# tsunrise/r1cs-spartan

Measured on AMD Instinct MI355X. Metric: R1CS constraints proved/sec at 2^20, higher is better.
Workload: dtype bls12-381 Fr/Fq Montgomery (u32 limbs)

## Files before the change

### include/spartan_hip.h

```cpp
#ifndef SPARTAN_HIP_H
#define SPARTAN_HIP_H
#include <stddef.h>
#include <stdint.h>

#ifdef __cplusplus
extern "C" {
#endif

typedef enum {
    SPX_OK = 0,
    SPX_INVALID_ARGUMENT = 1,
    SPX_SUMCHECK = 2,
    SPX_WRONG_WITNESS = 3,
    SPX_SERIALIZATION = 4,
    SPX_DEVICE = 5
} spx_status;

typedef struct spx_ctx spx_ctx;
typedef struct spx_pp spx_pp;
typedef struct spx_pk spx_pk;
typedef struct spx_witness spx_witness;

typedef struct {
    uint64_t n;
// ... 129 lines not shown
    SPX_K_RED_G1 = 11,
    SPX_K_RED_G2 = 12,
    SPX_K_COUNT = 13
};
int spx_kernel_stats_enable(spx_ctx *ctx, int on);
int spx_kernel_stats(spx_ctx *ctx, int id, uint64_t *launches, double *ms, double *bytes);
int spx_kernel_stats_largest(spx_ctx *ctx, int id, uint64_t *launches, double *ms, double *bytes);
int spx_kernel_ops(spx_ctx *ctx, int id, double *ops);
int spx_msm_reruns(spx_ctx *ctx, uint64_t *reruns);

int spx_msm_skew_stats(spx_ctx *ctx, uint64_t out[4]);

int spx_msm_window_plan(uint64_t size, int *c, int *windows);
int spx_msm_level_plan(int nv, int *c);
int spx_pp_window_plan(spx_pp *pp, int level, int *c, int *windows);

int spx_sum_over_y(spx_ctx *ctx, const spx_csr *m, const uint8_t *z, uint8_t *out);
int spx_eval_on_x(spx_ctx *ctx, const spx_csr *m, const uint8_t *r_x, uint8_t *out);
int spx_sumcheck_round(spx_ctx *ctx, const uint8_t *f, const uint8_t *g, size_t n, const uint8_t *r_prev,
                       uint8_t *evals_out, uint8_t *f_out, uint8_t *g_out);
int spx_msm_g1(spx_ctx *ctx, const uint8_t *bases, const uint8_t *scalars, size_t n, uint8_t *out96);
int spx_msm_g2(spx_ctx *ctx, const uint8_t *bases, const uint8_t *scalars, size_t n, uint8_t *out192);
int spx_g1_decompress(spx_ctx *ctx, const uint8_t *in, size_t n, uint8_t *out_uncompressed, uint8_t *ok);
int spx_g2_decompress(spx_ctx *ctx, const uint8_t *in, size_t n, uint8_t *out_uncompressed, uint8_t *ok);
int spx_lincomb_g1(spx_ctx *ctx, const uint8_t *bases_uncompressed, const uint8_t *scalars, size_t n,
                   const uint64_t *seg_off, size_t nseg, uint8_t *out_uncompressed);
int spx_lincomb_g2(spx_ctx *ctx, const uint8_t *bases_uncompressed, const uint8_t *scalars, size_t n,
                   const uint64_t *seg_off, size_t nseg, uint8_t *out_uncompressed);
int spx_g1_in_subgroup(spx_ctx *ctx, const uint8_t *pts_uncompressed, size_t n, uint8_t *ok);
int spx_g2_in_subgroup(spx_ctx *ctx, const uint8_t *pts_uncompressed, size_t n, uint8_t *ok);
// ... 16 lines not shown
```

### r1cs-spartan_amd/__init__.py

```python
import ctypes
import os

_HERE = os.path.dirname(os.path.abspath(__file__))
LIB_PATH = os.environ.get("SPX_LIB_PATH") or os.path.join(_HERE, "libspartan_hip.so")

R = 0x73EDA753299D7D483339D80809A1D80553BDA402FFFE5BFEFFFFFFFF00000001


class SpartanError(Exception):
    code = -1


class InvalidArgument(SpartanError):
    code = 1


class SumCheckError(SpartanError):
    code = 2


class WrongWitness(SpartanError):
    code = 3


# ... 41 lines not shown
    "spx_ctx_set_msm_hot",
    "spx_comm_hub_create_rccl",
    "spx_comm_hub_create_shm",
    "spx_comm_hub_create_group",
    "spx_comm_hub_create_callback",
    "spx_ctx_set_comm_hub",
    "spx_comm_hub_allgather",
    "spx_comm_hub_stats",
    "spx_comm_hub_destroy",
    "spx_ctx_comm_allgather",
    "spx_msm_reruns",
    "spx_msm_skew_stats",
    "spx_msm_window_plan",
    "spx_msm_level_plan",
    "spx_pp_window_plan",
    "spx_ctx_mem_info",
    "spx_ctx_set_sync_poll",
    "spx_ctx_set_group",
    "spx_host_phase_stats",
    "spx_pp_load",
    "spx_pp_generate",
    "spx_pp_serialize",
    "spx_pp_free",
    "spx_index",
    "spx_index_free",
    "spx_witness_upload",
    "spx_witness_free",
    "spx_proof_size",
    "spx_prove",
    "spx_prove_witness",
# ... 81 lines not shown
        L.spx_ctx_set_sync_poll.argtypes = [vp, ctypes.c_int]
    if hasattr(L, "spx_ctx_set_group") or not os.environ.get("SPX_LIB_PATH"):
        L.spx_ctx_set_group.argtypes = [vp, ctypes.c_int]
    if hasattr(L, "spx_ctx_mem_info") or not os.environ.get("SPX_LIB_PATH"):
        L.spx_ctx_mem_info.argtypes = [vp, ctypes.POINTER(ctypes.c_uint64), ctypes.POINTER(ctypes.c_uint64)]
    if hasattr(L, "spx_ctx_set_lvl0_batch"):
        L.spx_ctx_set_lvl0_batch.argtypes = [vp, ctypes.c_int]
    if hasattr(L, "spx_ctx_set_msm_hot") or not os.environ.get("SPX_LIB_PATH"):
        L.spx_ctx_set_msm_hot.argtypes = [vp, ctypes.c_int]
        L.spx_msm_skew_stats.argtypes = [vp, ctypes.POINTER(ctypes.c_uint64)]
    if hasattr(L, "spx_msm_window_plan") or not os.environ.get("SPX_LIB_PATH"):
        pint = ctypes.POINTER(ctypes.c_int)
        L.spx_msm_window_plan.argtypes = [ctypes.c_uint64, pint, pint]
        L.spx_msm_level_plan.argtypes = [ctypes.c_int, pint]
        L.spx_pp_window_plan.argtypes = [vp, ctypes.c_int, pint, pint]
    if hasattr(L, "spx_comm_hub_create_rccl") or not os.environ.get("SPX_LIB_PATH"):
        L.spx_comm_hub_create_rccl.argtypes = [u8p, ctypes.c_int, ctypes.c_int, ctypes.c_int, ctypes.POINTER(vp)]
        L.spx_comm_hub_create_shm.argtypes = [ctypes.c_char_p, ctypes.c_int, ctypes.c_int, ctypes.POINTER(vp)]
        L.spx_comm_hub_create_group.argtypes = [vp, ctypes.c_int, ctypes.POINTER(vp)]
        if hasattr(L, "spx_comm_hub_create_callback") or not os.environ.get("SPX_LIB_PATH"):
            L.spx_comm_hub_create_callback.argtypes = [ALLGATHER_FN, vp, ctypes.c_int, ctypes.c_int, ctypes.POINTER(vp)]
        L.spx_ctx_set_comm_hub.argtypes = [vp, vp, ctypes.c_int]
        L.spx_comm_hub_allgather.argtypes = [vp, ctypes.c_int, ctypes.c_char_p, ctypes.c_void_p, sz]
        L.spx_comm_hub_stats.argtypes = [vp, ctypes.c_void_p]
        L.spx_comm_hub_destroy.argtypes = [vp]
    L.spx_ctx_comm_allgather.argtypes = [vp, ctypes.c_char_p, ctypes.c_void_p, sz]
    L.spx_pp_load.argtypes = [vp, u8p, sz, ctypes.POINTER(vp)]
    L.spx_pp_generate.argtypes = [vp, ctypes.c_int, ctypes.c_uint64, ctypes.POINTER(vp)]
    L.spx_pp_serialize.argtypes = [vp, ctypes.c_void_p, sz, ctypes.POINTER(sz)]
    L.spx_pp_free.argtypes = [vp]
# ... 370 lines not shown
    def check_subgroup(self, strict=True):
        bad = ctypes.c_uint64(0)
        first = (ctypes.c_uint64 * 3)()
        rc = lib().spx_pp_check_subgroup(self.ctx.h, self.h, ctypes.byref(bad), first)
        if rc != 0 and (strict or rc != 4):
            _check(rc)
        if bad.value == 0:
            return 0, None
        return bad.value, (int(first[0]), None if first[1] == 2**64 - 1 else int(first[1]), int(first[2]))

    def window_plan(self, level):
        c, w = ctypes.c_int(0), ctypes.c_int(0)
        _check(lib().spx_pp_window_plan(self.h, int(level), ctypes.byref(c), ctypes.byref(w)))
        return c.value, w.value

    def serialize_uncompressed(self):
        n = ctypes.c_size_t(0)
        _check(lib().spx_pp_serialize(self.h, None, 0, ctypes.byref(n)))
        buf = ctypes.create_string_buffer(n.value)
        _check(lib().spx_pp_serialize(self.h, buf, n.value, ctypes.byref(n)))
        return buf.raw

    def __del__(self):
        try:
            if self.h and self.ctx.h:
                lib().spx_pp_free(self.h)
        except Exception:
            pass


# ... 479 lines not shown
```

### r1cs-spartan_amd/csrc/capi.cpp

```cpp
#include "../../include/spartan_hip.h"

#include <atomic>
#include <chrono>
#include <algorithm>
#include <cstdlib>
#include <mutex>
#include <condition_variable>
#include <memory>
#include <string>
#include <thread>
#include <vector>

#include "hash_sched.hpp"
#include "interactive.hpp"
#include "pairing.hpp"
#include "prover.hpp"

extern "C" int spx_comm_unique_id_impl(uint8_t out[128]);

struct spx_ctx {
    std::unique_ptr<spx::Ctx> c;
};
struct spx_pp {
    spx_ctx* ctx;
// ... 269 lines not shown
    });
}
int spx_pp_serialize(spx_pp* pp, uint8_t* out, size_t cap, size_t* len) {
    return guard([&] {
        set_dev(pp->ctx);
        copy_out(spx::pp_serialize(*pp->ctx->c, *pp->p), out, cap, len);
    });
}
int spx_pp_window_plan(spx_pp* pp, int level, int* c, int* windows) {
    return guard([&] {
        if (!pp || !c || !windows) spx::invalid("null argument");
        const spx::PP& P = *pp->p;
        if (level < -1 || level >= P.nv) spx::invalid("level out of range");
        *c = level < 0 ? P.g1_c : P.g2_c[level];
        *windows = level < 0 ? P.g1_W : P.g2_W[level];
    });
}
int spx_msm_window_plan(uint64_t size, int* c, int* windows) {
    return guard([&] {
        if (!c || !windows) spx::invalid("null argument");
        *c = spx::window_bits_for(size, spx::msm_wide_min_log());
        *windows = spx::windows_for(*c);
    });
}
int spx_msm_level_plan(int nv, int* c) {
    return guard([&] {
        if (!c) spx::invalid("null argument");
        if (nv < 1 || nv > spx::kMaxLogN) spx::invalid("nv out of range");
        const std::vector<int> plan = spx::g2_window_plan(nv, spx::msm_wide_min_log());
        std::copy(plan.begin(), plan.end(), c);
// ... 619 lines not shown
```

### r1cs-spartan_amd/csrc/curve_dev.hpp

```cpp
#pragma once
#include "ff_dev.hpp"

namespace spx {

template <class F>
struct Aff {
    F x, y;
};
template <class F>
struct Xyzz {
    F x, y, zz, zzz;
};
using G1Aff = Aff<Fq>;
struct G1Slot {
    G1Aff p;
    uint32_t pad[8];
};
static_assert(sizeof(G1Slot) == 128, "G1 table slot");
using G2Aff = Aff<Fq2>;
using G1Xyzz = Xyzz<Fq>;
using G2Xyzz = Xyzz<Fq2>;

template <class F>
DEV void xyzz_set_inf(Xyzz<F>& p) {
    FieldOps<F>::one(p.x);
    FieldOps<F>::one(p.y);
    FieldOps<F>::zero(p.zz);
    FieldOps<F>::zero(p.zzz);
}
template <class F>
DEV bool xyzz_is_inf(const Xyzz<F>& p) {
    return FieldOps<F>::is_zero(p.zz);
}

// ... 159 lines not shown
```

### r1cs-spartan_amd/csrc/kernels.hpp

```cpp
#pragma once
#include <hip/hip_runtime.h>
#include <stdint.h>

#include <vector>

#include "curve_dev.hpp"

namespace spx {

static constexpr uint64_t kLongRow = 64;
static constexpr uint64_t kChunk = 4096;

struct SparseView3 {
    const uint64_t* ptr[3];
    const uint32_t* idx[3];
    const Fr* val[3];
};
struct LongChunk {
    uint32_t m;
    uint32_t pad;
    uint64_t begin, end;
};
struct LongRow {
    uint32_t m;
// ... 202 lines not shown
static constexpr uint32_t kMsmOverflow = 1;
enum { kMsmStHot = 1, kMsmStReduced = 2, kMsmStLeafMax = 3 };

static constexpr uint64_t kMsmMaxBuckets = 2048ull << 8;
static constexpr uint32_t kMsmWideBits = 17, kMsmWideWindows = 15;
static constexpr uint32_t msm_windows(uint32_t c) { return c == kMsmWideBits ? kMsmWideWindows : (256 + c - 1) / c; }
struct MsmWorkspace;
MsmWorkspace* msm_ws_create();
void msm_ws_destroy(MsmWorkspace* ws);
void msm_ws_staging_reset(MsmWorkspace* ws);
void msm_ws_note_overflow(MsmWorkspace* ws);
void msm_ws_set_hot(MsmWorkspace* ws, bool on);
bool msm_hot_default();

inline size_t msm_out_bytes(bool g2, int ninst) { return (size_t)ninst * (g2 ? 4 * 96 : 4 * 48) + 16; }
void msm_run_g1(MsmWorkspace* ws, const MsmInst* insts_host, int ninst, const G1Slot* pts, const Fr* scalars,
                void* out_dev, hipStream_t s, const MsmShard& sh = MsmShard());
void msm_run_g2(MsmWorkspace* ws, const MsmInst* insts_host, int ninst, const G2Aff* pts, const Fr* scalars,
                void* out_dev, hipStream_t s, const MsmShard& sh = MsmShard());

void precompute_windows_g1(const G1Aff* raw, uint64_t count, bool pair_sum, int c, int W, G1Aff* dst, void* tmp,
                           hipStream_t s);
void precompute_windows_g2(const G2Aff* raw, uint64_t count, bool pair_sum, int c, int W, G2Aff* dst, void* tmp,
                           hipStream_t s);
void launch_points_from_bytes_g1(G1Aff* pts, uint64_t n, int* err, hipStream_t s);
void launch_points_from_bytes_g2(G2Aff* pts, uint64_t n, int* err, hipStream_t s);
void launch_points_to_canon_g1(G1Aff* pts, uint64_t n, hipStream_t s);
void launch_points_to_canon_g2(G2Aff* pts, uint64_t n, hipStream_t s);
void fixed_base_g1(const G1Aff* table, const Fr* scalars, uint64_t n, G1Aff* out, void* tmp, hipStream_t s);
void fixed_base_g2(const G2Aff* table, const Fr* scalars, uint64_t n, G2Aff* out, void* tmp, hipStream_t s);

void launch_decompress_g1(const uint8_t* in, uint64_t n, G1Aff* out, uint8_t* ok, hipStream_t s);
void launch_decompress_g2(const uint8_t* in, uint64_t n, G2Aff* out, uint8_t* ok, hipStream_t s);
size_t lincomb_tmp_bytes(bool g2, uint64_t n);
void launch_lincomb_g1(const G1Aff* pts, const Fr* scalars, uint64_t n, const uint64_t* seg_off, uint32_t nseg,
                       G1Aff* out, void* tmp, hipStream_t s);
void launch_lincomb_g2(const G2Aff* pts, const Fr* scalars, uint64_t n, const uint64_t* seg_off, uint32_t nseg,
                       G2Aff* out, void* tmp, hipStream_t s);

// ... 7 lines not shown
```

### r1cs-spartan_amd/csrc/msm_g1.hip

```cpp
#include "msm_impl.hpp"

namespace spx {

void msm_run_g1(MsmWorkspace* ws, const MsmInst* insts, int ninst, const G1Slot* pts, const Fr* scalars, void* out,
                hipStream_t s, const MsmShard& sh) {
    msm_run_t<Fq>(ws, insts, ninst, pts, scalars, out, s, sh);
}
void precompute_windows_g1(const G1Aff* raw, uint64_t count, bool pair_sum, int c, int W, G1Aff* dst, void* tmp,
                           hipStream_t s) {
    precompute_windows_t<Fq>(raw, count, pair_sum, c, W, dst, tmp, s);
}
void fixed_base_g1(const G1Aff* table, const Fr* scalars, uint64_t n, G1Aff* out, void* tmp, hipStream_t s) {
    fixed_base_t<Fq>(table, scalars, n, out, tmp, s);
}

}
```

### r1cs-spartan_amd/csrc/msm_g2.hip

```cpp
#include "msm_impl.hpp"

namespace spx {

void msm_run_g2(MsmWorkspace* ws, const MsmInst* insts, int ninst, const G2Aff* pts, const Fr* scalars, void* out,
                hipStream_t s, const MsmShard& sh) {
    msm_run_t<Fq2>(ws, insts, ninst, pts, scalars, out, s, sh);
}
void precompute_windows_g2(const G2Aff* raw, uint64_t count, bool pair_sum, int c, int W, G2Aff* dst, void* tmp,
                           hipStream_t s) {
    precompute_windows_t<Fq2>(raw, count, pair_sum, c, W, dst, tmp, s);
}
void fixed_base_g2(const G2Aff* table, const Fr* scalars, uint64_t n, G2Aff* out, void* tmp, hipStream_t s) {
    fixed_base_t<Fq2>(table, scalars, n, out, tmp, s);
}

}
```

### r1cs-spartan_amd/csrc/msm_impl.hpp

```cpp
#pragma once
#include "curve29.hpp"
#include "fq2pair.hpp"
#include "msm_common.hpp"

namespace spx {

template <class F>
struct Acc;
struct AffRaw {
    Fq x, y;
};
template <>
struct Acc<Fq> {
    using Pt = G1Slot;
    using T = F29;
    using TA = F29;
    static constexpr int kLanes = 1, kWaves = 1;
    static DEV void ld_raw(AffRaw& a, const G1Slot* p) { load_vec(*(Aff<Fq>*)&a, &p->p); }
    static DEV void unpack(T& x, T& y, const AffRaw& a) {
        f29_unpack(x, a.x.v);
        f29_unpack(y, a.y.v);
    }
    static DEV void ld_aff(T& x, T& y, const G1Slot* p) {
        AffRaw a;
        ld_raw(a, p);
        unpack(x, y, a);
    }
    static DEV bool aff_sentinel(const T& x, const T& y) { return f29_is_zero_raw(x) && f29_is_zero_raw(y); }
    static DEV void ld(X29<T>& r, const Xyzz<Fq>* p) { ld29<Fq>(r, p); }
    static DEV void st(Xyzz<Fq>* p, const X29<T>& r) { st29<Fq>(p, r); }
};
template <>
struct Acc<Fq2> {
    using Pt = Aff<Fq2>;
    using T = FP29;
    using TA = FP29A;
    static constexpr int kLanes = 2, kWaves = 2;
    static DEV void ld_raw(AffRaw& a, const Aff<Fq2>* p) {
        const bool odd = pair_odd();
        load_vec(a.x, odd ? &p->x.c1 : &p->x.c0);
        load_vec(a.y, odd ? &p->y.c1 : &p->y.c0);
    }
    template <class P>
    static DEV void unpack(P& x, P& y, const AffRaw& a) {
        f29_unpack(x.v, a.x.v);
        f29_unpack(y.v, a.y.v);
    }
    template <class P>
    static DEV void ld_aff(P& x, P& y, const Aff<Fq2>* p) {
        fp29_ld(x, &p->x);
        fp29_ld(y, &p->y);
    }
    template <class P>
    static DEV bool aff_sentinel(const P& x, const P& y) {
        return pair_all(f29_is_zero_raw(x.v) && f29_is_zero_raw(y.v));
    }
    static DEV void ld(X29<T>& r, const Xyzz<Fq2>* p) {
        fp29_ld(r.x, &p->x);
        fp29_ld(r.y, &p->y);
        fp29_ld(r.zz, &p->zz);
        fp29_ld(r.zzz, &p->zzz);
    }
    template <class P>
    static DEV void st(Xyzz<Fq2>* p, const X29<P>& r) {
        fp29_st(&p->x, r.x);
        fp29_st(&p->y, r.y);
        fp29_st(&p->zz, r.zz);
        fp29_st(&p->zzz, r.zzz);
    }
};
// ... 131 lines not shown
}
template <class F>
static unsigned tree_blocks(uint64_t elems) {
    return (unsigned)((elems * TreeLanes<F>::v + kHeavy - 1) / kHeavy);
}

template <class F>
DEV uint64_t acc_elem() {
    return (blockIdx.x * (uint64_t)blockDim.x + threadIdx.x) / Acc<F>::kLanes;
}
template <class F>
static unsigned acc_blocks(uint64_t elems) {
    return (unsigned)((elems * Acc<F>::kLanes + kHeavy - 1) / kHeavy);
}

template <class F>
__global__ __launch_bounds__(kHeavy, Acc<F>::kWaves) void k_accum_aff(const uint32_t* __restrict__ off, uint32_t nb,
                                                                      const uint32_t* __restrict__ pfx,
                                                                      const uint32_t* __restrict__ refs,
                                                                      const typename Acc<F>::Pt* __restrict__ pts,
                                                                      Xyzz<F>* __restrict__ out, uint32_t seg1) {
    using A = Acc<F>;
    using T = typename A::TA;
    const uint32_t t = (uint32_t)acc_elem<F>();
    const uint32_t total = off[nb];
    uint32_t e = t * seg1;
    if (e >= total) return;
    const uint32_t end = min(e + seg1, total);
    uint32_t b = find_bucket(off, nb, e);
    uint32_t bend = off[b + 1];
    uint32_t slot = pfx[b] + (t - off[b] / seg1);
    X29<T> acc;
    x29_set_inf(acc);
    for (; e < end; ++e) {
        if (e == bend) {
            A::st(out + slot, acc);
            x29_set_inf(acc);
            do {
                ++b;
            } while (off[b + 1] <= e);
            bend = off[b + 1];
            slot = pfx[b];
        }
        const uint32_t r = refs[e];
        T px, py;
        A::ld_aff(px, py, pts + (r & 0x7fffffffu));
        if (A::aff_sentinel(px, py)) continue;
        x29_madd(acc, px, py, (r >> 31) != 0);
    }
    A::st(out + slot, acc);
}

template <class F>
__global__ __launch_bounds__(kHeavy, Acc<F>::kWaves) void k_accum_xyzz(const uint32_t* __restrict__ segoff, uint32_t nb,
                                                                       const uint32_t* __restrict__ off,
                                                                       const Xyzz<F>* __restrict__ in,
                                                                       Xyzz<F>* __restrict__ out) {
    using A = Acc<F>;
    using T = typename A::T;
    const uint32_t s = (uint32_t)tree_elem<F>();
    if (s >= segoff[nb]) return;
    const uint32_t b = find_bucket(segoff, nb, s);
// ... 243 lines not shown
static int msm_levels_env() {
    static const int v = [] {
        const char* e = getenv("SPX_MSM_LEVELS");
        return e ? atoi(e) : -1;
    }();
    return v;
}
static int msm_seg1_env() {
    static const int v = [] {
        const char* e = getenv("SPX_MSM_SEG1");
        return e ? atoi(e) : 0;
    }();
    return v;
}

template <class F>
static void msm_run_t(MsmWorkspace* ws, const MsmInst* ih, int ninst, const typename Acc<F>::Pt* pts, const Fr* scalars,
                      void* out_dev, hipStream_t s, const MsmShard& sh) {
    if (ninst <= 0) return;
    const bool g2 = sizeof(F) == sizeof(Fq2);
    const size_t psz = sizeof(Xyzz<F>);
    const size_t ob = msm_out_bytes(g2, ninst);
    MsmPlan pl = msm_plan(ih, ninst, sh, ws->cap_scale);
    const int nact = (int)pl.insts.size();
    if (!nact) {
        HIPCHK(hipMemsetAsync(out_dev, 0, ob, s));
        return;
    }
    msm_upload_plan(ws, pl, s);
    const uint32_t nb = pl.nb;
    const uint64_t tot_refs = pl.tot_refs;
    uint32_t kSeg1 = seg1_fit(seg1_len(g2), tot_refs, Acc<F>::kWaves, Acc<F>::kLanes);
    if (msm_seg1_env() > 0) kSeg1 = std::min<uint32_t>(kSeg1, (uint32_t)msm_seg1_env());
    const double mu = pl.mu_max;
    int nlev = 0;
    for (uint32_t m = (uint32_t)std::ceil((mu + 6.0 * std::sqrt(mu) + 16.0) / kSeg1) + 1; m > 1; m = (m + kSeg - 1) / kSeg)
        ++nlev;
    if (msm_levels_env() >= 0) nlev = std::min(nlev, msm_levels_env());
    MsmSorted so = msm_sort(ws, pl, scalars, out_dev, ob, s, kSeg1, nlev);
    const uint64_t max_segs = tot_refs / kSeg1 + nb + 1;
    auto* PA = (Xyzz<F>*)ws->pa.ensure(psz * max_segs);
    auto* PB = (Xyzz<F>*)ws->pb.ensure(psz * (max_segs / kSeg + nb + 1));
    uint32_t* cur_off = so.np_off;
    uint32_t* nxt_off = nullptr;
    const uint64_t nthr = (tot_refs + kSeg1 - 1) / kSeg1;
    kp_begin(g2 ? KP_ACC_G2 : KP_ACC_G1, s);
    hipLaunchKernelGGL(k_accum_aff<F>, dim3(acc_blocks<F>(nthr)), dim3(kHeavy), 0, s, so.offs, nb, cur_off, so.refs, pts, PA,
                       kSeg1);
    kp_end((double)tot_refs * (4.0 + sizeof(Aff<F>)) + (double)(tot_refs / kSeg1) * psz, s, (double)tot_refs);
    Xyzz<F>* cur = PA;
    Xyzz<F>* nxt = PB;
    uint64_t cur_max_segs = max_segs;
    for (int l = 0; l < nlev; ++l) {
        nxt_off = so.lev[l];
        uint64_t nsegs = cur_max_segs / kSeg + nb + 1;
        kp_begin(g2 ? KP_ACCX_G2 : KP_ACCX_G1, s);
        hipLaunchKernelGGL(k_accum_xyzz<F>, dim3(tree_blocks<F>(nsegs)), dim3(kHeavy), 0, s, nxt_off, nb, cur_off, cur, nxt);
        kp_end((double)(cur_max_segs + nsegs) * psz, s, (double)cur_max_segs);
        std::swap(cur, nxt);
        std::swap(cur_off, nxt_off);
        cur_max_segs = nsegs;
    }
// ... 98 lines not shown
            continue;
        }
        F d, di, izz, izzz;
        O::mul(di, inv, out[k].x);
        O::mul(d, p.zz, p.zzz);
        O::mul(inv, inv, d);
        O::mul(izz, di, p.zzz);
        O::mul(izzz, di, p.zz);
        Aff<F> a;
        O::mul(a.x, p.x, izz);
        O::mul(a.y, p.y, izzz);
        store_vec(out + k, a);
    }
}

template <class F>
__global__ __launch_bounds__(kHeavy) void k_aff_to_r29(Aff<F>* __restrict__ a, uint64_t n) {
    using T = typename R29<F>::T;
    const uint64_t j = blockIdx.x * (uint64_t)blockDim.x + threadIdx.x;
    if (j >= n) return;
    Aff<F> p;
    load_vec(p, a + j);
    T x, y, mx, my;
    R29<F>::unpack(x, p.x);
    R29<F>::unpack(y, p.y);
    f29_map(mx, x, Q29::FROM_R1);
    f29_map(my, y, Q29::FROM_R1);
    R29<F>::pack(p.x, mx);
    R29<F>::pack(p.y, my);
    store_vec(a + j, p);
}

template <class F>
static void precompute_windows_t(const Aff<F>* raw, uint64_t count, bool pair_sum, int c, int W, Aff<F>* dst, void* tmp,
                               hipStream_t s) {
    if (!count) return;
    Xyzz<F>* t = (Xyzz<F>*)tmp;
    hipLaunchKernelGGL(k_precompute<F>, dim3((unsigned)((count + kHeavy - 1) / kHeavy)), dim3(kHeavy), 0, s, raw, count,
                       pair_sum ? 1 : 0, c, W, t);
    const uint64_t n = count * (uint64_t)W;
    const uint64_t nt = (n + kNormChunk - 1) / kNormChunk;
    hipLaunchKernelGGL(k_normalize<F>, dim3((unsigned)((nt + kHeavy - 1) / kHeavy)), dim3(kHeavy), 0, s, t, n, dst);
    hipLaunchKernelGGL(k_aff_to_r29<F>, dim3((unsigned)((n + kHeavy - 1) / kHeavy)), dim3(kHeavy), 0, s, dst, n);
    HIPCHK(hipGetLastError());
}
template <class F>
__global__ __launch_bounds__(kHeavy) void k_fixed_base(const Aff<F>* __restrict__ table, const Fr* __restrict__ scalars,
                                                       uint64_t n, Xyzz<F>* __restrict__ tmp) {
    const uint64_t j = blockIdx.x * (uint64_t)blockDim.x + threadIdx.x;
    if (j >= n) return;
    Fr m, s;
    load_vec(m, scalars + j);
    fe_from_mont(s, m);
    Xyzz<F> acc;
    xyzz_set_inf(acc);
    for (int w = 0; w < 32; ++w) {
        const uint32_t d = (s.v[w >> 2] >> (8 * (w & 3))) & 0xffu;
        if (d) {
// ... 19 lines not shown
```

### r1cs-spartan_amd/csrc/prover.cpp

```cpp
#include "prover.hpp"
#include "sc_message.hpp"
#include "pairing.hpp"

#include <type_traits>

#include <algorithm>
#include <sys/prctl.h>

#include <chrono>
#include <thread>
#include <cstdlib>
#include <cstring>

namespace spx {

using host::Affine;
using HFr = host::Fr;
using HFq = host::Fq;
using HFq2 = host::Fq2;

Ctx::Ctx(int dev) : device(dev) {
    static const bool blocking = [] {
        const char* e = getenv("SPX_BLOCKING_SYNC");
        return e && e[0] == '1';
// ... 116 lines not shown
    for (int i = 0; i < nv; ++i) {
        c[i] = window_bits_for(1ull << (nv - i - 1), 0);
        buckets += 1ull << (c[i] - 1);
    }
    for (int i = 0; i < nv; ++i) {
        const int cw = window_bits_for(1ull << (nv - i - 1), wide_min_log);
        if (cw == c[i]) break;
        const uint64_t with = buckets - (1ull << (c[i] - 1)) + (1ull << (cw - 1));
        if (with > kMsmMaxBuckets) break;
        c[i] = cw;
        buckets = with;
    }
    return c;
}

template <class A, class D>
static void precompute_level(Ctx& C, const A* raw, uint64_t count, bool pair, int c, int W, D* dst) {
    const uint64_t chunk = std::min<uint64_t>(count, 1ull << 18);
    const size_t xyzz_sz = 2 * sizeof(A);
    DevMem tmp(xyzz_sz * chunk * W), aff(sizeof(A) * chunk * W);
    for (uint64_t j0 = 0; j0 < count; j0 += chunk) {
        const uint64_t cn = std::min(chunk, count - j0);
        const A* src = raw + (pair ? 2 * j0 : j0);
        if constexpr (sizeof(A) == sizeof(G1Aff))
            precompute_windows_g1((const G1Aff*)src, cn, pair, c, W, aff.as<G1Aff>(), tmp.p, C.stream);
        else
            precompute_windows_g2((const G2Aff*)src, cn, pair, c, W, aff.as<G2Aff>(), tmp.p, C.stream);
        if constexpr (sizeof(D) == sizeof(A)) {
            SPX_HIP(hipMemcpy2DAsync(dst + j0, sizeof(A) * count, aff.p, sizeof(A) * cn, sizeof(A) * cn, W,
                                     hipMemcpyDeviceToDevice, C.stream));
        } else {
            for (int w = 0; w < W; ++w)
                SPX_HIP(hipMemcpy2DAsync(dst + (uint64_t)w * count + j0, sizeof(D), aff.as<A>() + (uint64_t)w * cn,
                                         sizeof(A), sizeof(A), cn, hipMemcpyDeviceToDevice, C.stream));
        }
    }
    C.sync();
}

void pp_preprocess(Ctx& C, PP& P) {
    const int nv = P.nv;
    const uint64_t n = 1ull << nv;
    const int wide = msm_wide_min_log();
    P.g1_c = window_bits_for(n, wide);
    P.g1_W = windows_for(P.g1_c);
    P.g1_pre.alloc(sizeof(G1Slot) * n * P.g1_W);
    precompute_level(C, P.g1_level(0), n, false, P.g1_c, P.g1_W, P.g1_pre.as<G1Slot>());
    P.g2_off.assign(nv + 1, 0);
    P.g2_c = g2_window_plan(nv, wide);
    P.g2_W.assign(nv, 0);
    uint64_t tot = 0;
    for (int i = 0; i < nv; ++i) {
        uint64_t cnt = 1ull << (nv - i - 1);
        P.g2_W[i] = windows_for(P.g2_c[i]);
        P.g2_off[i] = tot;
        tot += cnt * P.g2_W[i];
    }
    P.g2_off[nv] = tot;
    P.g2_pre.alloc(sizeof(G2Aff) * std::max<uint64_t>(tot, 1));
    for (int i = 0; i < nv; ++i) {
        uint64_t cnt = 1ull << (nv - i - 1);
        precompute_level(C, P.g2_level(i), cnt, true, P.g2_c[i], P.g2_W[i], P.g2_pre.as<G2Aff>() + P.g2_off[i]);
    }
}

static void pp_alloc_raw(PP& P, int nv) {
    P.nv = nv;
    P.lvl_off.assign(nv + 1, 0);
    uint64_t tot = 0;
    for (int i = 0; i < nv; ++i) {
        P.lvl_off[i] = tot;
        tot += 1ull << (nv - i);
    }
    P.lvl_off[nv] = tot;
    P.g1_raw_mem.alloc(sizeof(G1Aff) * std::max<uint64_t>(tot, 1));
    P.g2_raw_mem.alloc(sizeof(G2Aff) * std::max<uint64_t>(tot, 1));
}
// ... 725 lines not shown
        st = C.side;
        ws = C.msm_side;
        g_kprof = nullptr;
    }
    Fr* q = C.buf<Fr>(Ctx::kSlotLvl0Q, 32 * half);
    launch_open_level(z, nullptr, q, Fr{}, half, st);
    MsmInst I{};
    I.pts_off = P.g2_off[0];
    I.stride = (uint32_t)half;
    I.scalar_off = 0;
    I.size = (uint32_t)half;
    I.c = (uint32_t)P.g2_c[0];
    I.W = (uint32_t)P.g2_W[0];
    const size_t ob = msm_out_bytes(true, 1);
    void* out = C.buf(Ctx::kSlotLvl0Out, ob);
    msm_run_g2(ws, &I, 1, P.g2_pre.as<G2Aff>(), q, out, st, sh);
    SPX_HIP(hipMemcpyAsync(C.pin_at(Ctx::kPinLvl0, ob, 4 << 10), out, ob, hipMemcpyDeviceToHost, st));
}
static Affine<HFq2> lvl0_finish(Ctx& C, PP& P, const Fr* z, int L, Comm& comm, bool on_side = false) {
    if (on_side)
        C.side_sync();
    else
        C.sync();
    const uint8_t* h = C.pin_at(Ctx::kPinLvl0, msm_out_bytes(true, 1), 4 << 10);
    if (msm_status(h, true, 1) & kMsmOverflow) {
        msm_ws_note_overflow(on_side ? C.msm_side : C.msm);
        ++C.msm_reruns;
        MsmShard sh = shard_of(comm);
        sh.dense = true;
        lvl0_launch(C, P, z, L, sh, on_side);
        if (on_side)
// ... 61 lines not shown
        I.stride = (uint32_t)half;
        I.scalar_off = qoff;
        I.size = (uint32_t)half;
        I.c = (uint32_t)P.g2_c[i];
        I.W = (uint32_t)P.g2_W[i];
        qoff += half;
    }
    const int nm = L - first;
    const size_t ob = msm_out_bytes(true, nm);
    void* out = C.buf(Ctx::kSlotOpenOut, ob);
    uint8_t* h = C.pin_at(Ctx::kPinOpen, ob + 32, 56 << 10);
    for (int attempt = 0;; ++attempt) {
        MsmShard sh = shard_of(comm);
        sh.dense = attempt > 0;
        if (nm) {
            msm_run_g2(C.msm, insts.data(), nm, P.g2_pre.as<G2Aff>(), q, out, C.stream, sh);
            SPX_HIP(hipMemcpyAsync(h, out, ob, hipMemcpyDeviceToHost, C.stream));
        }
        if (!attempt) SPX_HIP(hipMemcpyAsync(h + ob, rin, 32, hipMemcpyDeviceToHost, C.stream));
        C.sync();
        if (!nm || !(msm_status(h, true, nm) & kMsmOverflow)) break;
        msm_ws_note_overflow(C.msm);
        ++C.msm_reruns;
    }
    if (nm) msm_skew_fold(C, h, true, nm);
    res.eval = ld_hfr(h + ob);
    std::vector<Affine<HFq2>> part = msm_results<HFq2>(comm, h, nm);
    for (int k = 0; k < nm; ++k) res.proofs[first + k] = part[k];
    return res;
}

// ... 1865 lines not shown
    const size_t ps = g2 ? 192 : 96;
    DevMem raw(ps * n), sc(32 * n), err(sizeof(int));
    SPX_HIP(hipMemsetAsync(err.p, 0, 4, C.stream));
    SPX_HIP(hipMemcpyAsync(raw.p, bases, ps * n, hipMemcpyHostToDevice, C.stream));
    SPX_HIP(hipMemcpyAsync(sc.p, scalars, 32 * n, hipMemcpyHostToDevice, C.stream));
    launch_to_mont(sc.as<Fr>(), n, err.as<int>(), C.stream);
    if (g2)
        launch_points_from_bytes_g2(raw.as<G2Aff>(), n, err.as<int>(), C.stream);
    else
        launch_points_from_bytes_g1(raw.as<G1Aff>(), n, err.as<int>(), C.stream);
    MsmInst I{};
    I.c = (uint32_t)window_bits_for(n, msm_wide_min_log());
    I.W = (uint32_t)windows_for((int)I.c);
    I.size = (uint32_t)n;
    I.stride = (uint32_t)n;
    DevMem pre((g2 ? sizeof(G2Aff) : sizeof(G1Slot)) * n * I.W), out(msm_out_bytes(g2, 1));
    if (g2)
        precompute_level(C, raw.as<G2Aff>(), n, false, (int)I.c, (int)I.W, pre.as<G2Aff>());
    else
        precompute_level(C, raw.as<G1Aff>(), n, false, (int)I.c, (int)I.W, pre.as<G1Slot>());
    if (g2)
        msm_run_g2(C.msm, &I, 1, pre.as<G2Aff>(), sc.as<Fr>(), out.p, C.stream);
    else
        msm_run_g1(C.msm, &I, 1, pre.as<G1Slot>(), sc.as<Fr>(), out.p, C.stream);
    std::vector<uint8_t> h(out.bytes);
    int herr = 0;
    SPX_HIP(hipMemcpyAsync(h.data(), out.p, out.bytes, hipMemcpyDeviceToHost, C.stream));
    SPX_HIP(hipMemcpyAsync(&herr, err.p, 4, hipMemcpyDeviceToHost, C.stream));
    C.sync();
    if (herr & 1) throw SpxError(kSerialization, "non-canonical input");
    if (herr & 2) throw SpxError(kSerialization, "base point not on the curve");
    msm_skew_fold(C, h.data(), g2, 1);
    std::vector<uint8_t> res(ps);
    LocalComm local;
    if (g2)
        host::g2_to_uncompressed(res.data(), msm_results<HFq2>(local, h.data(), 1)[0]);
    else
// ... 32 lines not shown
```

### r1cs-spartan_amd/csrc/prover.hpp

```cpp
#pragma once
#include <hip/hip_runtime.h>

#include <algorithm>
#include <atomic>
#include <chrono>
#include <cstdlib>
#include <cstring>
#include <condition_variable>
#include <functional>
#include <memory>
#include <mutex>
#include <thread>
#include <stdexcept>
#include <string>
#include <vector>

#include "host_ff.hpp"
#include "kernels.hpp"
#include "transcript.hpp"

namespace spx {

struct SpxError : std::runtime_error {
    int code;
// ... 222 lines not shown
    void release() {
        if (c) c->in_use.store(false);
        c = nullptr;
    }
};

struct PP {
    int nv = 0;
    DevMem g1_raw_mem, g2_raw_mem;
    std::vector<uint64_t> lvl_off;
    host::Affine<host::Fq> g;
    host::Affine<host::Fq2> h;
    DevMem g1_pre;
    int g1_c = 0, g1_W = 0;
    DevMem g2_pre;
    std::vector<uint64_t> g2_off;
    std::vector<int> g2_c, g2_W;
    bool has_t = false;
    std::vector<host::Fr> t;
    G1Aff* g1_level(int i) const { return g1_raw_mem.as<G1Aff>() + lvl_off[i]; }
    G2Aff* g2_level(int i) const { return g2_raw_mem.as<G2Aff>() + lvl_off[i]; }
};
void pp_preprocess(Ctx& C, PP& P);
int window_bits_for(uint64_t size, int wide_min_log);
int windows_for(int c);
int msm_wide_min_log();
std::vector<int> g2_window_plan(int nv, int wide_min_log);

struct HostCsr {
    uint64_t n = 0;
    std::vector<uint64_t> rp;
    std::vector<uint32_t> col;
    std::vector<uint8_t> val;
};
struct DevSparse {
    DevMem ptr[3], idx[3], val[3];
    DevMem chunks, lrows;
    int nchunks = 0, nlrows = 0;
    SparseView3 view() const {
        SparseView3 v;
        for (int m = 0; m < 3; ++m) {
// ... 120 lines not shown
```

Before: 64.79 million.

## Store MSM base tables in unpacked 29-bit limb form, add optional G2 limb table

```diff
diff --git a/include/spartan_hip.h b/include/spartan_hip.h
--- a/include/spartan_hip.h
+++ b/include/spartan_hip.h
@@ -167,6 +167,7 @@
 int spx_msm_window_plan(uint64_t size, int *c, int *windows);
 int spx_msm_level_plan(int nv, int *c);
 int spx_pp_window_plan(spx_pp *pp, int level, int *c, int *windows);
+int spx_pp_table_form(spx_pp *pp, int *g2_limb);
 
 int spx_sum_over_y(spx_ctx *ctx, const spx_csr *m, const uint8_t *z, uint8_t *out);
 int spx_eval_on_x(spx_ctx *ctx, const spx_csr *m, const uint8_t *r_x, uint8_t *out);
diff --git a/r1cs-spartan_amd/__init__.py b/r1cs-spartan_amd/__init__.py
--- a/r1cs-spartan_amd/__init__.py
+++ b/r1cs-spartan_amd/__init__.py
@@ -79,6 +79,7 @@
     "spx_msm_window_plan",
     "spx_msm_level_plan",
     "spx_pp_window_plan",
+    "spx_pp_table_form",
     "spx_ctx_mem_info",
     "spx_ctx_set_sync_poll",
     "spx_ctx_set_group",
@@ -190,6 +191,8 @@
         L.spx_msm_window_plan.argtypes = [ctypes.c_uint64, pint, pint]
         L.spx_msm_level_plan.argtypes = [ctypes.c_int, pint]
         L.spx_pp_window_plan.argtypes = [vp, ctypes.c_int, pint, pint]
+        if hasattr(L, "spx_pp_table_form") or not os.environ.get("SPX_LIB_PATH"):
+            L.spx_pp_table_form.argtypes = [vp, pint]
     if hasattr(L, "spx_comm_hub_create_rccl") or not os.environ.get("SPX_LIB_PATH"):
         L.spx_comm_hub_create_rccl.argtypes = [u8p, ctypes.c_int, ctypes.c_int, ctypes.c_int, ctypes.POINTER(vp)]
         L.spx_comm_hub_create_shm.argtypes = [ctypes.c_char_p, ctypes.c_int, ctypes.c_int, ctypes.POINTER(vp)]
@@ -590,6 +593,11 @@
         _check(lib().spx_pp_window_plan(self.h, int(level), ctypes.byref(c), ctypes.byref(w)))
         return c.value, w.value
 
+    def table_form(self):
+        v = ctypes.c_int(0)
+        _check(lib().spx_pp_table_form(self.h, ctypes.byref(v)))
+        return "limb" if v.value else "packed"
+
     def serialize_uncompressed(self):
         n = ctypes.c_size_t(0)
         _check(lib().spx_pp_serialize(self.h, None, 0, ctypes.byref(n)))
diff --git a/r1cs-spartan_amd/csrc/capi.cpp b/r1cs-spartan_amd/csrc/capi.cpp
--- a/r1cs-spartan_amd/csrc/capi.cpp
+++ b/r1cs-spartan_amd/csrc/capi.cpp
@@ -307,6 +307,12 @@
         if (level < -1 || level >= P.nv) spx::invalid("level out of range");
         *c = level < 0 ? P.g1_c : P.g2_c[level];
         *windows = level < 0 ? P.g1_W : P.g2_W[level];
+    });
+}
+int spx_pp_table_form(spx_pp* pp, int* g2_limb) {
+    return guard([&] {
+        if (!pp || !g2_limb) spx::invalid("null argument");
+        *g2_limb = pp->p->g2_limb ? 1 : 0;
     });
 }
 int spx_msm_window_plan(uint64_t size, int* c, int* windows) {
diff --git a/r1cs-spartan_amd/csrc/curve_dev.hpp b/r1cs-spartan_amd/csrc/curve_dev.hpp
--- a/r1cs-spartan_amd/csrc/curve_dev.hpp
+++ b/r1cs-spartan_amd/csrc/curve_dev.hpp
@@ -12,12 +12,18 @@
     F x, y, zz, zzz;
 };
 using G1Aff = Aff<Fq>;
-struct G1Slot {
-    G1Aff p;
-    uint32_t pad[8];
+struct alignas(16) LimbSlot {
+    uint32_t x[14], y[14];
+    uint32_t pad[4];
 };
+static constexpr uint32_t kSlotInf = 1u << 31;
+using G1Slot = LimbSlot;
 static_assert(sizeof(G1Slot) == 128, "G1 table slot");
 using G2Aff = Aff<Fq2>;
+struct G2Slot {
+    LimbSlot h[2];
+};
+static_assert(sizeof(G2Slot) == 256, "G2 limb-form table slot");
 using G1Xyzz = Xyzz<Fq>;
 using G2Xyzz = Xyzz<Fq2>;
 
diff --git a/r1cs-spartan_amd/csrc/kernels.hpp b/r1cs-spartan_amd/csrc/kernels.hpp
--- a/r1cs-spartan_amd/csrc/kernels.hpp
+++ b/r1cs-spartan_amd/csrc/kernels.hpp
@@ -240,15 +240,21 @@
 bool msm_hot_default();
 
 inline size_t msm_out_bytes(bool g2, int ninst) { return (size_t)ninst * (g2 ? 4 * 96 : 4 * 48) + 16; }
+struct G2Table {
+    void* p = nullptr;
+    bool limb = false;
+    static size_t elem_bytes(bool limb) { return limb ? sizeof(G2Slot) : sizeof(G2Aff); }
+    G2Table at(uint64_t i) const { return G2Table{(uint8_t*)p + i * elem_bytes(limb), limb}; }
+};
 void msm_run_g1(MsmWorkspace* ws, const MsmInst* insts_host, int ninst, const G1Slot* pts, const Fr* scalars,
                 void* out_dev, hipStream_t s, const MsmShard& sh = MsmShard());
-void msm_run_g2(MsmWorkspace* ws, const MsmInst* insts_host, int ninst, const G2Aff* pts, const Fr* scalars,
+void msm_run_g2(MsmWorkspace* ws, const MsmInst* insts_host, int ninst, G2Table pts, const Fr* scalars,
                 void* out_dev, hipStream_t s, const MsmShard& sh = MsmShard());
 
-void precompute_windows_g1(const G1Aff* raw, uint64_t count, bool pair_sum, int c, int W, G1Aff* dst, void* tmp,
-                           hipStream_t s);
-void precompute_windows_g2(const G2Aff* raw, uint64_t count, bool pair_sum, int c, int W, G2Aff* dst, void* tmp,
-                           hipStream_t s);
+void precompute_windows_g1(const G1Aff* raw, uint64_t count, bool pair_sum, int c, int W, G1Aff* aff, void* tmp,
+                           G1Slot* dst, uint64_t pitch, hipStream_t s);
+void precompute_windows_g2(const G2Aff* raw, uint64_t count, bool pair_sum, int c, int W, G2Aff* aff, void* tmp,
+                           G2Table dst, uint64_t pitch, hipStream_t s);
 void launch_points_from_bytes_g1(G1Aff* pts, uint64_t n, int* err, hipStream_t s);
 void launch_points_from_bytes_g2(G2Aff* pts, uint64_t n, int* err, hipStream_t s);
 void launch_points_to_canon_g1(G1Aff* pts, uint64_t n, hipStream_t s);
diff --git a/r1cs-spartan_amd/csrc/msm_g1.hip b/r1cs-spartan_amd/csrc/msm_g1.hip
--- a/r1cs-spartan_amd/csrc/msm_g1.hip
+++ b/r1cs-spartan_amd/csrc/msm_g1.hip
@@ -4,11 +4,11 @@
 
 void msm_run_g1(MsmWorkspace* ws, const MsmInst* insts, int ninst, const G1Slot* pts, const Fr* scalars, void* out,
                 hipStream_t s, const MsmShard& sh) {
-    msm_run_t<Fq>(ws, insts, ninst, pts, scalars, out, s, sh);
+    msm_run_t<Fq, G1Slot>(ws, insts, ninst, pts, scalars, out, s, sh);
 }
-void precompute_windows_g1(const G1Aff* raw, uint64_t count, bool pair_sum, int c, int W, G1Aff* dst, void* tmp,
-                           hipStream_t s) {
-    precompute_windows_t<Fq>(raw, count, pair_sum, c, W, dst, tmp, s);
+void precompute_windows_g1(const G1Aff* raw, uint64_t count, bool pair_sum, int c, int W, G1Aff* aff, void* tmp,
+                           G1Slot* dst, uint64_t pitch, hipStream_t s) {
+    precompute_windows_t<Fq, G1Slot>(raw, count, pair_sum, c, W, aff, tmp, dst, pitch, s);
 }
 void fixed_base_g1(const G1Aff* table, const Fr* scalars, uint64_t n, G1Aff* out, void* tmp, hipStream_t s) {
     fixed_base_t<Fq>(table, scalars, n, out, tmp, s);
diff --git a/r1cs-spartan_amd/csrc/msm_g2.hip b/r1cs-spartan_amd/csrc/msm_g2.hip
--- a/r1cs-spartan_amd/csrc/msm_g2.hip
+++ b/r1cs-spartan_amd/csrc/msm_g2.hip
@@ -2,13 +2,19 @@
 
 namespace spx {
 
-void msm_run_g2(MsmWorkspace* ws, const MsmInst* insts, int ninst, const G2Aff* pts, const Fr* scalars, void* out,
+void msm_run_g2(MsmWorkspace* ws, const MsmInst* insts, int ninst, G2Table pts, const Fr* scalars, void* out,
                 hipStream_t s, const MsmShard& sh) {
-    msm_run_t<Fq2>(ws, insts, ninst, pts, scalars, out, s, sh);
+    if (pts.limb)
+        msm_run_t<Fq2, G2Slot>(ws, insts, ninst, (const G2Slot*)pts.p, scalars, out, s, sh);
+    else
+        msm_run_t<Fq2, G2Aff>(ws, insts, ninst, (const G2Aff*)pts.p, scalars, out, s, sh);
 }
-void precompute_windows_g2(const G2Aff* raw, uint64_t count, bool pair_sum, int c, int W, G2Aff* dst, void* tmp,
-                           hipStream_t s) {
-    precompute_windows_t<Fq2>(raw, count, pair_sum, c, W, dst, tmp, s);
+void precompute_windows_g2(const G2Aff* raw, uint64_t count, bool pair_sum, int c, int W, G2Aff* aff, void* tmp,
+                           G2Table dst, uint64_t pitch, hipStream_t s) {
+    if (dst.limb)
+        precompute_windows_t<Fq2, G2Slot>(raw, count, pair_sum, c, W, aff, tmp, (G2Slot*)dst.p, pitch, s);
+    else
+        precompute_windows_t<Fq2, G2Aff>(raw, count, pair_sum, c, W, aff, tmp, (G2Aff*)dst.p, pitch, s);
 }
 void fixed_base_g2(const G2Aff* table, const Fr* scalars, uint64_t n, G2Aff* out, void* tmp, hipStream_t s) {
     fixed_base_t<Fq2>(table, scalars, n, out, tmp, s);
diff --git a/r1cs-spartan_amd/csrc/msm_impl.hpp b/r1cs-spartan_amd/csrc/msm_impl.hpp
--- a/r1cs-spartan_amd/csrc/msm_impl.hpp
+++ b/r1cs-spartan_amd/csrc/msm_impl.hpp
@@ -7,53 +7,64 @@
 
 template <class F>
 struct Acc;
-struct AffRaw {
-    Fq x, y;
+struct SlotXY {
+    uint32_t x[14], y[14];
 };
+DEV void slot_ld(F29& x, F29& y, const LimbSlot* p) {
+    SlotXY a;
+    load_vec(a, (const SlotXY*)p);
+#pragma unroll
+    for (int i = 0; i < 14; ++i) {
+        x.v[i] = a.x[i];
+        y.v[i] = a.y[i];
+    }
+}
+DEV bool slot_inf(const F29& x) { return (x.v[13] & kSlotInf) != 0; }
+DEV void slot_st(LimbSlot* p, const F29& x, const F29& y, bool inf) {
+    LimbSlot a;
+#pragma unroll
+    for (int i = 0; i < 14; ++i) {
+        a.x[i] = x.v[i];
+        a.y[i] = y.v[i];
+    }
+    if (inf) a.x[13] |= kSlotInf;
+#pragma unroll
+    for (int i = 0; i < 4; ++i) a.pad[i] = 0;
+    store_vec(p, a);
+}
 template <>
 struct Acc<Fq> {
-    using Pt = G1Slot;
     using T = F29;
     using TA = F29;
     static constexpr int kLanes = 1, kWaves = 1;
-    static DEV void ld_raw(AffRaw& a, const G1Slot* p) { load_vec(*(Aff<Fq>*)&a, &p->p); }
-    static DEV void unpack(T& x, T& y, const AffRaw& a) {
-        f29_unpack(x, a.x.v);
-        f29_unpack(y, a.y.v);
-    }
-    static DEV void ld_aff(T& x, T& y, const G1Slot* p) {
-        AffRaw a;
-        ld_raw(a, p);
-        unpack(x, y, a);
-    }
-    static DEV bool aff_sentinel(const T& x, const T& y) { return f29_is_zero_raw(x) && f29_is_zero_raw(y); }
+    static DEV void ld_aff(T& x, T& y, const G1Slot* p) { slot_ld(x, y, p); }
+    template <class Tab>
+    static DEV bool aff_sentinel(const T& x, const T&) {
+        return slot_inf(x);
+    }
     static DEV void ld(X29<T>& r, const Xyzz<Fq>* p) { ld29<Fq>(r, p); }
     static DEV void st(Xyzz<Fq>* p, const X29<T>& r) { st29<Fq>(p, r); }
 };
 template <>
 struct Acc<Fq2> {
-    using Pt = Aff<Fq2>;
     using T = FP29;
     using TA = FP29A;
     static constexpr int kLanes = 2, kWaves = 2;
-    static DEV void ld_raw(AffRaw& a, const Aff<Fq2>* p) {
-        const bool odd = pair_odd();
-        load_vec(a.x, odd ? &p->x.c1 : &p->x.c0);
-        load_vec(a.y, odd ? &p->y.c1 : &p->y.c0);
-    }
-    template <class P>
-    static DEV void unpack(P& x, P& y, const AffRaw& a) {
-        f29_unpack(x.v, a.x.v);
-        f29_unpack(y.v, a.y.v);
-    }
     template <class P>
     static DEV void ld_aff(P& x, P& y, const Aff<Fq2>* p) {
         fp29_ld(x, &p->x);
         fp29_ld(y, &p->y);
     }
     template <class P>
+    static DEV void ld_aff(P& x, P& y, const G2Slot* p) {
+        slot_ld(x.v, y.v, &p->h[pair_odd() ? 1 : 0]);
+    }
+    template <class Tab, class P>
     static DEV bool aff_sentinel(const P& x, const P& y) {
-        return pair_all(f29_is_zero_raw(x.v) && f29_is_zero_raw(y.v));
+        if constexpr (sizeof(Tab) == sizeof(G2Slot))
+            return slot_inf(x.v);
+        else
+            return pair_all(f29_is_zero_raw(x.v) && f29_is_zero_raw(y.v));
     }
     static DEV void ld(X29<T>& r, const Xyzz<Fq2>* p) {
         fp29_ld(r.x, &p->x);
@@ -215,11 +226,11 @@
     return (unsigned)((elems * Acc<F>::kLanes + kHeavy - 1) / kHeavy);
 }
 
-template <class F>
+template <class F, class Pt>
 __global__ __launch_bounds__(kHeavy, Acc<F>::kWaves) void k_accum_aff(const uint32_t* __restrict__ off, uint32_t nb,
                                                                       const uint32_t* __restrict__ pfx,
                                                                       const uint32_t* __restrict__ refs,
-                                                                      const typename Acc<F>::Pt* __restrict__ pts,
+                                                                      const Pt* __restrict__ pts,
                                                                       Xyzz<F>* __restrict__ out, uint32_t seg1) {
     using A = Acc<F>;
     using T = typename A::TA;
@@ -246,7 +257,7 @@
         const uint32_t r = refs[e];
         T px, py;
         A::ld_aff(px, py, pts + (r & 0x7fffffffu));
-        if (A::aff_sentinel(px, py)) continue;
+        if (A::template aff_sentinel<Pt>(px, py)) continue;
         x29_madd(acc, px, py, (r >> 31) != 0);
     }
     A::st(out + slot, acc);
@@ -520,8 +531,8 @@
     return v;
 }
 
-template <class F>
-static void msm_run_t(MsmWorkspace* ws, const MsmInst* ih, int ninst, const typename Acc<F>::Pt* pts, const Fr* scalars,
+template <class F, class Pt>
+static void msm_run_t(MsmWorkspace* ws, const MsmInst* ih, int ninst, const Pt* pts, const Fr* scalars,
                       void* out_dev, hipStream_t s, const MsmShard& sh) {
     if (ninst <= 0) return;
     const bool g2 = sizeof(F) == sizeof(Fq2);
@@ -551,7 +562,7 @@
     uint32_t* nxt_off = nullptr;
     const uint64_t nthr = (tot_refs + kSeg1 - 1) / kSeg1;
     kp_begin(g2 ? KP_ACC_G2 : KP_ACC_G1, s);
-    hipLaunchKernelGGL(k_accum_aff<F>, dim3(acc_blocks<F>(nthr)), dim3(kHeavy), 0, s, so.offs, nb, cur_off, so.refs, pts, PA,
+    hipLaunchKernelGGL((k_accum_aff<F, Pt>), dim3(acc_blocks<F>(nthr)), dim3(kHeavy), 0, s, so.offs, nb, cur_off, so.refs, pts, PA,
                        kSeg1);
     kp_end((double)tot_refs * (4.0 + sizeof(Aff<F>)) + (double)(tot_refs / kSeg1) * psz, s, (double)tot_refs);
     Xyzz<F>* cur = PA;
@@ -680,8 +691,20 @@
     }
 }
 
-template <class F>
-__global__ __launch_bounds__(kHeavy) void k_aff_to_r29(Aff<F>* __restrict__ a, uint64_t n) {
+DEV void tab_st(G1Slot* d, const F29& x, const F29& y, bool inf) { slot_st(d, x, y, inf); }
+DEV void tab_st(G2Slot* d, const F2_29& x, const F2_29& y, bool inf) {
+    slot_st(&d->h[0], x.c0, y.c0, inf);
+    slot_st(&d->h[1], x.c1, y.c1, inf);
+}
+DEV void tab_st(Aff<Fq2>* d, const F2_29& x, const F2_29& y, bool) {
+    Aff<Fq2> p;
+    R29<Fq2>::pack(p.x, x);
+    R29<Fq2>::pack(p.y, y);
+    store_vec(d, p);
+}
+template <class F, class Pt>
+__global__ __launch_bounds__(kHeavy) void k_aff_to_table(const Aff<F>* __restrict__ a, uint64_t n, uint64_t cn,
+                                                         Pt* __restrict__ dst, uint64_t pitch) {
     using T = typename R29<F>::T;
     const uint64_t j = blockIdx.x * (uint64_t)blockDim.x + threadIdx.x;
     if (j >= n) return;
@@ -692,22 +715,21 @@
     R29<F>::unpack(y, p.y);
     f29_map(mx, x, Q29::FROM_R1);
     f29_map(my, y, Q29::FROM_R1);
-    R29<F>::pack(p.x, mx);
-    R29<F>::pack(p.y, my);
-    store_vec(a + j, p);
-}
-
-template <class F>
-static void precompute_windows_t(const Aff<F>* raw, uint64_t count, bool pair_sum, int c, int W, Aff<F>* dst, void* tmp,
-                               hipStream_t s) {
+    tab_st(dst + (j / cn) * pitch + j % cn, mx, my, aff_is_sentinel(p));
+}
+
+template <class F, class Pt>
+static void precompute_windows_t(const Aff<F>* raw, uint64_t count, bool pair_sum, int c, int W, Aff<F>* aff, void* tmp,
+                                 Pt* dst, uint64_t pitch, hipStream_t s) {
     if (!count) return;
     Xyzz<F>* t = (Xyzz<F>*)tmp;
     hipLaunchKernelGGL(k_precompute<F>, dim3((unsigned)((count + kHeavy - 1) / kHeavy)), dim3(kHeavy), 0, s, raw, count,
                        pair_sum ? 1 : 0, c, W, t);
     const uint64_t n = count * (uint64_t)W;
     const uint64_t nt = (n + kNormChunk - 1) / kNormChunk;
-    hipLaunchKernelGGL(k_normalize<F>, dim3((unsigned)((nt + kHeavy - 1) / kHeavy)), dim3(kHeavy), 0, s, t, n, dst);
-    hipLaunchKernelGGL(k_aff_to_r29<F>, dim3((unsigned)((n + kHeavy - 1) / kHeavy)), dim3(kHeavy), 0, s, dst, n);
+    hipLaunchKernelGGL(k_normalize<F>, dim3((unsigned)((nt + kHeavy - 1) / kHeavy)), dim3(kHeavy), 0, s, t, n, aff);
+    hipLaunchKernelGGL((k_aff_to_table<F, Pt>), dim3((unsigned)((n + kHeavy - 1) / kHeavy)), dim3(kHeavy), 0, s, aff, n,
+                       count, dst, pitch);
     HIPCHK(hipGetLastError());
 }
 template <class F>
diff --git a/r1cs-spartan_amd/csrc/prover.cpp b/r1cs-spartan_amd/csrc/prover.cpp
--- a/r1cs-spartan_amd/csrc/prover.cpp
+++ b/r1cs-spartan_amd/csrc/prover.cpp
@@ -154,8 +154,15 @@
     return c;
 }
 
+bool g2_table_limb() {
+    const char* e = getenv("SPX_MSM_G2_TABLE");
+    if (!e || !*e || !strcmp(e, "packed")) return false;
+    if (!strcmp(e, "limb")) return true;
+    throw SpxError(kInvalidArgument, "SPX_MSM_G2_TABLE: limb or packed");
+}
+
 template <class A, class D>
-static void precompute_level(Ctx& C, const A* raw, uint64_t count, bool pair, int c, int W, D* dst) {
+static void precompute_level(Ctx& C, const A* raw, uint64_t count, bool pair, int c, int W, D dst) {
     const uint64_t chunk = std::min<uint64_t>(count, 1ull << 18);
     const size_t xyzz_sz = 2 * sizeof(A);
     DevMem tmp(xyzz_sz * chunk * W), aff(sizeof(A) * chunk * W);
@@ -163,17 +170,9 @@
         const uint64_t cn = std::min(chunk, count - j0);
         const A* src = raw + (pair ? 2 * j0 : j0);
         if constexpr (sizeof(A) == sizeof(G1Aff))
-            precompute_windows_g1((const G1Aff*)src, cn, pair, c, W, aff.as<G1Aff>(), tmp.p, C.stream);
+            precompute_windows_g1((const G1Aff*)src, cn, pair, c, W, aff.as<G1Aff>(), tmp.p, dst + j0, count, C.stream);
         else
-            precompute_windows_g2((const G2Aff*)src, cn, pair, c, W, aff.as<G2Aff>(), tmp.p, C.stream);
-        if constexpr (sizeof(D) == sizeof(A)) {
-            SPX_HIP(hipMemcpy2DAsync(dst + j0, sizeof(A) * count, aff.p, sizeof(A) * cn, sizeof(A) * cn, W,
-                                     hipMemcpyDeviceToDevice, C.stream));
-        } else {
-            for (int w = 0; w < W; ++w)
-                SPX_HIP(hipMemcpy2DAsync(dst + (uint64_t)w * count + j0, sizeof(D), aff.as<A>() + (uint64_t)w * cn,
-                                         sizeof(A), sizeof(A), cn, hipMemcpyDeviceToDevice, C.stream));
-        }
+            precompute_windows_g2((const G2Aff*)src, cn, pair, c, W, aff.as<G2Aff>(), tmp.p, dst.at(j0), count, C.stream);
     }
     C.sync();
 }
@@ -182,6 +181,7 @@
     const int nv = P.nv;
     const uint64_t n = 1ull << nv;
     const int wide = msm_wide_min_log();
+    P.g2_limb = g2_table_limb();
     P.g1_c = window_bits_for(n, wide);
     P.g1_W = windows_for(P.g1_c);
     P.g1_pre.alloc(sizeof(G1Slot) * n * P.g1_W);
@@ -197,10 +197,10 @@
         tot += cnt * P.g2_W[i];
     }
     P.g2_off[nv] = tot;
-    P.g2_pre.alloc(sizeof(G2Aff) * std::max<uint64_t>(tot, 1));
+    P.g2_pre.alloc(G2Table::elem_bytes(P.g2_limb) * std::max<uint64_t>(tot, 1));
     for (int i = 0; i < nv; ++i) {
         uint64_t cnt = 1ull << (nv - i - 1);
-        precompute_level(C, P.g2_level(i), cnt, true, P.g2_c[i], P.g2_W[i], P.g2_pre.as<G2Aff>() + P.g2_off[i]);
+        precompute_level(C, P.g2_level(i), cnt, true, P.g2_c[i], P.g2_W[i], P.g2_table().at(P.g2_off[i]));
     }
 }
 
@@ -956,7 +956,7 @@
     I.W = (uint32_t)P.g2_W[0];
     const size_t ob = msm_out_bytes(true, 1);
     void* out = C.buf(Ctx::kSlotLvl0Out, ob);
-    msm_run_g2(ws, &I, 1, P.g2_pre.as<G2Aff>(), q, out, st, sh);
+    msm_run_g2(ws, &I, 1, P.g2_table(), q, out, st, sh);
     SPX_HIP(hipMemcpyAsync(C.pin_at(Ctx::kPinLvl0, ob, 4 << 10), out, ob, hipMemcpyDeviceToHost, st));
 }
 static Affine<HFq2> lvl0_finish(Ctx& C, PP& P, const Fr* z, int L, Comm& comm, bool on_side = false) {
@@ -1048,7 +1048,7 @@
         MsmShard sh = shard_of(comm);
         sh.dense = attempt > 0;
         if (nm) {
-            msm_run_g2(C.msm, insts.data(), nm, P.g2_pre.as<G2Aff>(), q, out, C.stream, sh);
+            msm_run_g2(C.msm, insts.data(), nm, P.g2_table(), q, out, C.stream, sh);
             SPX_HIP(hipMemcpyAsync(h, out, ob, hipMemcpyDeviceToHost, C.stream));
         }
         if (!attempt) SPX_HIP(hipMemcpyAsync(h + ob, rin, 32, hipMemcpyDeviceToHost, C.stream));
@@ -2944,13 +2944,15 @@
     I.W = (uint32_t)windows_for((int)I.c);
     I.size = (uint32_t)n;
     I.stride = (uint32_t)n;
-    DevMem pre((g2 ? sizeof(G2Aff) : sizeof(G1Slot)) * n * I.W), out(msm_out_bytes(g2, 1));
+    const bool limb = g2 && g2_table_limb();
+    DevMem pre((g2 ? G2Table::elem_bytes(limb) : sizeof(G1Slot)) * n * I.W), out(msm_out_bytes(g2, 1));
+    const G2Table tab2{pre.p, limb};
     if (g2)
-        precompute_level(C, raw.as<G2Aff>(), n, false, (int)I.c, (int)I.W, pre.as<G2Aff>());
+        precompute_level(C, raw.as<G2Aff>(), n, false, (int)I.c, (int)I.W, tab2);
     else
         precompute_level(C, raw.as<G1Aff>(), n, false, (int)I.c, (int)I.W, pre.as<G1Slot>());
     if (g2)
-        msm_run_g2(C.msm, &I, 1, pre.as<G2Aff>(), sc.as<Fr>(), out.p, C.stream);
+        msm_run_g2(C.msm, &I, 1, tab2, sc.as<Fr>(), out.p, C.stream);
     else
         msm_run_g1(C.msm, &I, 1, pre.as<G1Slot>(), sc.as<Fr>(), out.p, C.stream);
     std::vector<uint8_t> h(out.bytes);
diff --git a/r1cs-spartan_amd/csrc/prover.hpp b/r1cs-spartan_amd/csrc/prover.hpp
--- a/r1cs-spartan_amd/csrc/prover.hpp
+++ b/r1cs-spartan_amd/csrc/prover.hpp
@@ -260,6 +260,8 @@
     DevMem g1_pre;
     int g1_c = 0, g1_W = 0;
     DevMem g2_pre;
+    bool g2_limb = false;
+    G2Table g2_table() const { return G2Table{g2_pre.p, g2_limb}; }
     std::vector<uint64_t> g2_off;
     std::vector<int> g2_c, g2_W;
     bool has_t = false;
@@ -271,6 +273,7 @@
 int window_bits_for(uint64_t size, int wide_min_log);
 int windows_for(int c);
 int msm_wide_min_log();
+bool g2_table_limb();
 std::vector<int> g2_window_plan(int nv, int wide_min_log);
 
 struct HostCsr {
```

After: 64.77 million. About the same (-0.0%).
